# RioWong/PointCloudProcess

Hardware: AMD Instinct MI355X
Metric: Mcorrespondences/s + ICP iter/s, 50M-vs-50M fp32 @ 1/2/4/8 MI355X (higher is better)
Workload: dtype f32

## Files before the change

include/pcp.h:

```cpp
#ifndef PCP_H
#define PCP_H

#include <stddef.h>
#include <stdint.h>

#ifdef __cplusplus
extern "C" {
#endif

#define PCP_ABI_VERSION 1

enum pcp_status {
    PCP_OK = 0,
    PCP_ERR_ARG = -1,
    PCP_ERR_HIP = -2,
    PCP_ERR_NOMEM = -3,
    PCP_ERR_EMPTY = -4,
    PCP_ERR_UNSUPPORTED = -5,
    PCP_ERR_ICP = -6,
    PCP_ERR_CAPACITY = -7
};

#define PCP_AOS48_STRIDE 48

// ... 121 lines not shown
#define PCP_ICP_ABLATE_NO_FALLBACK 8
#define PCP_ICP_ABLATE_NO_VERIFY 64
#define PCP_ICP_OPT_WIDE_CACHE 128
#define PCP_ICP_OPT_GRAPH 256
#define PCP_ICP_OPT_NO_LOOKAHEAD 512
int pcp_icp_set_options(pcp_icp* icp, int oct_lanes_first, int oct_lanes_list, int ring_lanes, int ablate);
int pcp_icp_destroy(pcp_icp* icp);
int pcp_icp_step(pcp_ctx* ctx, pcp_icp* icp, const double T_host[16], float rmax,
                 double* acc_dev, int32_t* corr_idx_dev, float* corr_d2_dev);
int pcp_icp_keys(pcp_ctx* ctx, pcp_icp* icp, const double T_host[16], float rmax,
                 int64_t target_offset, uint64_t* keys_dev);
int pcp_icp_accumulate_keys(pcp_ctx* ctx, pcp_icp* icp, const double T_host[16],
                            const uint64_t* keys_dev, int64_t lo, int64_t hi,
                            const float* shard_xyz_dev, size_t shard_stride_bytes,
                            double* acc_dev);
int pcp_icp_keys_dev(pcp_ctx* ctx, pcp_icp* icp, const double* T_dev, float rmax,
                     int64_t target_offset, uint64_t* keys_dev);
int pcp_keys_owner(pcp_ctx* ctx, const uint64_t* keys_dev, int64_t n, const int64_t* bounds_dev, int nshards,
                   uint8_t* owner_dev);
int pcp_icp_accumulate_owned(pcp_ctx* ctx, const double* T_dev, const float* q_dev, size_t q_stride_bytes,
                             int64_t nq, const uint64_t* keys_dev, const uint8_t* owner_dev, int rank,
                             int64_t lo, int64_t hi, const float* shard_xyz_dev, size_t shard_stride_bytes,
                             double* acc_dev);
int pcp_slab_guard(pcp_ctx* ctx, const double* T_dev, const double box_host[6], double lo,
                   double hi, int* flag_dev);
int pcp_icp_solve(const double acc_host[24], int do_scale, double dT_host[16]);
int pcp_icp_run(pcp_ctx* ctx, pcp_icp* icp, double T_inout[16], float rmax, int iters,
                int do_scale, double eps, float* err);
int pcp_icp_last_kernel_ms(const pcp_icp* icp, double* ms, int* launches);
int pcp_icp_step_dev(pcp_ctx* ctx, pcp_icp* icp, const double* T_dev, float rmax, double* acc_dev);
int pcp_icp_solve_dev(pcp_ctx* ctx, const double* acc_dev, int do_scale, double* T_dev, double* stats_dev);
int pcp_icp_run_dev(pcp_ctx* ctx, pcp_icp* icp, double* T_dev, float rmax, int iters, int do_scale,
                    double* stats_dev);
int pcp_icp_kernel_ms(pcp_ctx* ctx, pcp_icp* icp, double* ms, int* launches);
int pcp_icp_last_fallback(const pcp_icp* icp, int64_t* n);
int pcp_icp_last_searched(const pcp_icp* icp, int64_t* n);
int pcp_icp_last_lookahead(const pcp_icp* icp, double* beta, double* max_offset_m);

int pcp_get_rot_icp(pcp_ctx* ctx, const void* src_aos48_dev, int64_t ns, int src_is_dense,
                    const void* temp_aos48_dev, int64_t nt, int temp_is_dense,
                    double mat_rot_host[16], float rmax, int iters, int do_scale,
                    double cell_size, float* err);

#define PCP_ICP_PLANE_ACC 30
typedef struct pcp_icp_planes pcp_icp_planes;

int pcp_icp_planes_create(pcp_ctx* ctx, const float* target_xyz_dev, size_t t_stride_bytes,
                          const float* normals_dev, size_t n_stride_bytes, int64_t n,
                          pcp_icp_planes** out);
int pcp_icp_planes_destroy(pcp_icp_planes* planes);
int64_t pcp_icp_planes_size(const pcp_icp_planes* planes);
int64_t pcp_icp_planes_valid(const pcp_icp_planes* planes);

int pcp_icp_accumulate_plane(pcp_ctx* ctx, const double* T_dev, const float* q_dev, size_t q_stride_bytes,
                             int64_t nq, const uint64_t* keys_dev, const pcp_icp_planes* planes,
                             double* acc_dev );
int pcp_icp_solve_plane(const double acc_host[30], double dT_host[16]);
int pcp_icp_solve_plane_dev(pcp_ctx* ctx, const double* acc_dev, double* T_dev, double* stats_dev );
int pcp_icp_run_plane_dev(pcp_ctx* ctx, pcp_icp* icp, const pcp_icp_planes* planes, const float* q_dev,
                          size_t q_stride_bytes, int64_t nq, double* T_dev, float rmax, int iters,
                          double* stats_dev);
int pcp_get_rot_icp_plane(pcp_ctx* ctx, const void* src_aos48_dev, int64_t ns, int src_is_dense,
                          const void* temp_aos48_dev, int64_t nt, int temp_is_dense,
                          double mat_rot_host[16], float rmax, int iters, int normals_k,
                          double cell_size, float* err);

// ... 75 lines not shown
```

pointcloudprocess_amd/_lib.py:

```python
import ctypes as C
import os

HERE = os.path.dirname(os.path.abspath(__file__))
_AB = os.environ.get("PCP_AB") == "1" and bool(os.environ.get("PCP_LIB"))
LIB_PATH = os.environ["PCP_LIB"] if _AB else os.path.join(HERE, "libpcp.so")

PCP_OK = 0
_STATUS = {
    -1: "PCP_ERR_ARG", -2: "PCP_ERR_HIP", -3: "PCP_ERR_NOMEM", -4: "PCP_ERR_EMPTY",
    -5: "PCP_ERR_UNSUPPORTED", -6: "PCP_ERR_ICP", -7: "PCP_ERR_CAPACITY",
}

_vp, _i32, _i64, _sz, _f32, _f64, _u32 = (C.c_void_p, C.c_int, C.c_int64, C.c_size_t,
                                          C.c_float, C.c_double, C.c_uint32)
_P = C.POINTER
SIGNATURES = [
    ("pcp_abi_version", _i32, []),
    ("pcp_ctx_create", _i32, [_i32, _vp, _P(_vp)]),
    ("pcp_ctx_destroy", _i32, [_vp]),
    ("pcp_ctx_set_stream", _i32, [_vp, _vp]),
    ("pcp_ctx_stream", _vp, [_vp]),
    ("pcp_last_error", C.c_char_p, [_vp]),
    ("pcp_sync", _i32, [_vp]),
    ("pcp_ctx_alloc_stats", _i32, [_vp, _vp]),
# ... 38 lines not shown
    ("pcp_grid_create", _i32, [_vp, _P(_vp)]),
    ("pcp_grid_destroy", _i32, [_vp]),
    ("pcp_grid_clear", _i32, [_vp, _vp]),
    ("pcp_grid_add_cloud", _i32, [_vp, _vp, _vp, _i64]),
    ("pcp_grid_size", _i64, [_vp]),
    ("pcp_grid_cells", _i64, [_vp]),
    ("pcp_grid_last_dedupe", _i32, [_vp, _P(_i64)]),
    ("pcp_grid_points", _i32, [_vp, _vp, _vp, _i64, _P(_i64)]),
    ("pcp_grid_box", _i32, [_vp, _vp, _i32, _i32, _i32, _i32, _vp, _i64, _P(_i64)]),
    ("pcp_grid_match", _i32, [_vp, _vp, _vp, _i64, _f32, _vp, _P(_i64), _vp, _i64, _P(_i64)]),
    ("pcp_pose_lum_elch", _i32, [_vp, _i64, _i64, _i64, _vp]),
    ("pcp_pose_loop_closure", _i32, [_vp, _vp, _i64, _vp, _vp, _i64, _i64]),
    ("pcp_remove_duplicate", _i32, [_vp, _vp, _i64, _i32, _f32, _vp, _P(_i64)]),
    ("pcp_normals_knn", _i32, [_vp, _vp, _i32, _vp, _i64]),
    ("pcp_normals_knn_last_deferred", _i32, [_vp, _P(_i64), _P(_i64)]),
    ("pcp_icp_create", _i32, [_vp, _vp, _vp, _sz, _i64, _P(_vp)]),
    ("pcp_icp_check_sizes", _i32, [_i64, _i64]),
    ("pcp_icp_destroy", _i32, [_vp]),
    ("pcp_icp_create_with_target", _i32, [_vp, _vp, _sz, _i64, _f64, _vp, _sz, _i64, _P(_vp), _P(_vp)]),
    ("pcp_icp_set_options", _i32, [_vp, _i32, _i32, _i32, _i32]),
    ("pcp_icp_step", _i32, [_vp, _vp, _P(_f64), _f32, _vp, _vp, _vp]),
    ("pcp_icp_keys", _i32, [_vp, _vp, _P(_f64), _f32, _i64, _vp]),
    ("pcp_icp_accumulate_keys", _i32, [_vp, _vp, _P(_f64), _vp, _i64, _i64, _vp, _sz, _vp]),
    ("pcp_icp_keys_dev", _i32, [_vp, _vp, _vp, _f32, _i64, _vp]),
    ("pcp_keys_owner", _i32, [_vp, _vp, _i64, _vp, _i32, _vp]),
    ("pcp_icp_accumulate_owned", _i32, [_vp, _vp, _vp, _sz, _i64, _vp, _vp, _i32, _i64, _i64, _vp, _sz, _vp]),
    ("pcp_slab_guard", _i32, [_vp, _vp, _P(_f64), _f64, _f64, _vp]),
    ("pcp_icp_solve", _i32, [_P(_f64), _i32, _P(_f64)]),
    ("pcp_icp_run", _i32, [_vp, _vp, _P(_f64), _f32, _i32, _i32, _f64, _P(_f32)]),
    ("pcp_icp_last_kernel_ms", _i32, [_vp, _P(_f64), _P(_i32)]),
    ("pcp_icp_step_dev", _i32, [_vp, _vp, _vp, _f32, _vp]),
    ("pcp_icp_solve_dev", _i32, [_vp, _vp, _i32, _vp, _vp]),
    ("pcp_icp_run_dev", _i32, [_vp, _vp, _vp, _f32, _i32, _i32, _vp]),
    ("pcp_icp_kernel_ms", _i32, [_vp, _vp, _P(_f64), _P(_i32)]),
    ("pcp_icp_last_fallback", _i32, [_vp, _P(_i64)]),
    ("pcp_icp_last_searched", _i32, [_vp, _P(_i64)]),
    ("pcp_icp_last_lookahead", _i32, [_vp, _P(_f64), _P(_f64)]),
    ("pcp_fault_report_install", _i32, []),
    ("pcp_build_id", C.c_char_p, []),
    ("pcp_get_rot_icp", _i32, [_vp, _vp, _i64, _i32, _vp, _i64, _i32, _P(_f64), _f32, _i32, _i32,
                               _f64, _P(_f32)]),
    ("pcp_icp_planes_create", _i32, [_vp, _vp, _sz, _vp, _sz, _i64, _P(_vp)]),
    ("pcp_icp_planes_destroy", _i32, [_vp]),
    ("pcp_icp_planes_size", _i64, [_vp]),
    ("pcp_icp_planes_valid", _i64, [_vp]),
    ("pcp_icp_accumulate_plane", _i32, [_vp, _vp, _vp, _sz, _i64, _vp, _vp, _vp]),
    ("pcp_icp_solve_plane", _i32, [_P(_f64), _P(_f64)]),
    ("pcp_icp_solve_plane_dev", _i32, [_vp, _vp, _vp, _vp]),
    ("pcp_icp_run_plane_dev", _i32, [_vp, _vp, _vp, _vp, _sz, _i64, _vp, _f32, _i32, _vp]),
    ("pcp_get_rot_icp_plane", _i32, [_vp, _vp, _i64, _i32, _vp, _i64, _i32, _P(_f64), _f32, _i32, _i32,
                                     _f64, _P(_f32)]),
    ("pcp_icp_trim_keys", _i32, [_vp, _vp, _i64, _f32, _f32, _f32, _vp, _vp]),
    ("pcp_icp_run_plane_trimmed_dev", _i32, [_vp, _vp, _vp, _vp, _sz, _i64, _vp, _f32, _f32, _f32, _f32, _i32,
                                             _vp, _vp]),
    ("pcp_get_rot_icp_plane_trimmed", _i32, [_vp, _vp, _i64, _i32, _vp, _i64, _i32, _P(_f64), _f32, _f32, _f32,
                                             _f32, _i32, _i32, _f64, _P(_f32), _P(_i64)]),
    ("pcp_icp_trim_keys_plane", _i32, [_vp, _vp, _vp, _sz, _i64, _vp, _vp, _f32, _f32, _f32, _vp, _vp]),
    ("pcp_icp_run_plane_rtrimmed_dev", _i32, [_vp, _vp, _vp, _vp, _sz, _i64, _vp, _f32, _f32, _f32, _f32, _i32,
                                              _vp, _vp]),
    ("pcp_get_rot_icp_plane_rtrimmed", _i32, [_vp, _vp, _i64, _i32, _vp, _i64, _i32, _P(_f64), _f32, _f32, _f32,
                                              _f32, _i32, _i32, _f64, _P(_f32), _P(_i64)]),
    ("pcp_icp_batch_create", _i32, [_vp, _vp, _vp, _sz, _i64, _P(_i64), _i32, _P(_vp)]),
    ("pcp_icp_batch_destroy", _i32, [_vp]),
    ("pcp_icp_batch_queries", _i64, [_vp]),
    ("pcp_icp_batch_segments", _i32, [_vp]),
    ("pcp_icp_batch_keys_dev", _i32, [_vp, _vp, _vp, _f32, _vp]),
# ... 54 lines not shown
```

pointcloudprocess_amd/csrc/icp.hip:

```cpp
#include <cmath>
#include <cstdlib>
#include <cstring>
#include <vector>

#include <rocprim/device/device_select.hpp>
#include <rocprim/iterator/counting_iterator.hpp>
#include "sortcfg.hpp"

#include "icp_pair.hpp"
#include "wave_acc.hpp"

namespace pcp {
struct QXyz {
    float x, y, z;
};
}

struct pcp_icp {
    pcp_ctx* ctx = nullptr;
    pcp_ctx* owner = nullptr;
    const pcp_index* target = nullptr;
    int64_t nq = 0;
    int64_t nq_in = 0;
    pcp::QXyz* q = nullptr;
// ... 1037 lines not shown
        ring_run<2>(a, s_acc, list, list_n);
    else if (G == 4)
        ring_run<4>(a, s_acc, list, list_n);
    else
        ring_run<8>(a, s_acc, list, list_n);
    write_wave_partials(s_acc, partials + (int64_t)blockIdx.x * kAcc);
}

__global__ void __launch_bounds__(256) k_list_compact(const int32_t* __restrict__ seg, const uint32_t* __restrict__ cnt,
                                                      int64_t nseg, int64_t seg_cap, int32_t* __restrict__ out,
                                                      uint32_t* __restrict__ total) {
    __shared__ uint32_t s_part[4];
    const int lane = threadIdx.x & 63, w = threadIdx.x >> 6;
    const int64_t s0 = (int64_t)blockIdx.x * 4;
    uint32_t acc = 0;
    for (int64_t i = threadIdx.x; i < s0; i += 256) acc += cnt[i];
    for (int o = 32; o > 0; o >>= 1) acc += (uint32_t)__shfl_xor((int)acc, o, 64);
    if (lane == 0) s_part[w] = acc;
    __syncthreads();
    const uint32_t base = s_part[0] + s_part[1] + s_part[2] + s_part[3];
    uint32_t c[4];
#pragma unroll
    for (int k = 0; k < 4; k++) c[k] = s0 + k < nseg ? cnt[s0 + k] : 0u;
    uint32_t off = base;
#pragma unroll
    for (int k = 0; k < 3; k++) off += k < w ? c[k] : 0u;
    const int64_t sg = s0 + w;
    if (sg < nseg)
        for (uint32_t k = (uint32_t)lane; k < c[w]; k += 64) out[off + k] = seg[sg * seg_cap + k];
    if (s0 + 4 >= nseg && threadIdx.x == 0) *total = base + c[0] + c[1] + c[2] + c[3];
}

constexpr int kRedGroups = 32;
__global__ void __launch_bounds__(kAcc * kRedGroups) k_reduce_partials(const double* __restrict__ part, int nb,
                                                                       double* out, const uint32_t* fb_total) {
    __shared__ double s[kRedGroups][kAcc];
    const int k = threadIdx.x % kAcc, grp = threadIdx.x / kAcc;
    double v = 0.0;
    int b = grp;
    for (; b + 7 * kRedGroups < nb; b += 8 * kRedGroups) {
        double x[8];
#pragma unroll
        for (int u = 0; u < 8; u++) x[u] = part[(int64_t)(b + u * kRedGroups) * kAcc + k];
#pragma unroll
        for (int u = 0; u < 8; u++) v += x[u];
    }
    for (; b < nb; b += kRedGroups) v += part[(int64_t)b * kAcc + k];
    s[grp][k] = v;
    __syncthreads();
    if (threadIdx.x < kAcc) {
        double t = 0.0;
        for (int j = 0; j < kRedGroups; j++) t += s[j][threadIdx.x];
        out[threadIdx.x] = threadIdx.x == kAcc - 1 ? (fb_total ? (double)*fb_total : 0.0) : t;
    }
}

__global__ void k_scatter_corr(IcpArgs a, int32_t* idx, float* d2) {
    load_pose(a);
    for (int64_t i = blockIdx.x * (int64_t)blockDim.x + threadIdx.x; i < a.nq;
         i += (int64_t)gridDim.x * blockDim.x) {
        const float4 qq = ldq(a, i);
        const int oq = a.qidx[i];
        float x, y, z;
        xform(a, qq, x, y, z);
        const CacheBest w = cache_best(a.tp, cache_load(a, i), x, y, z);
        const bool ok = w.bd <= a.r2;
        idx[oq] = ok ? w.bj : -1;
        d2[oq] = ok ? w.bd : INFINITY;
    }
}

__global__ void k_fill_corr(int32_t* idx, float* d2, int64_t n) {
    for (int64_t i = blockIdx.x * (int64_t)blockDim.x + threadIdx.x; i < n;
         i += (int64_t)gridDim.x * blockDim.x) {
        idx[i] = -1;
        d2[i] = INFINITY;
    }
}

__global__ void k_fill_keys(uint64_t* keys, int64_t n) {
    for (int64_t i = blockIdx.x * (int64_t)blockDim.x + threadIdx.x; i < n; i += (int64_t)gridDim.x * blockDim.x)
        keys[i] = kNoKey;
}

__global__ void k_make_keys(IcpArgs a, uint32_t offset, uint64_t* keys) {
    load_pose(a);
    for (int64_t i = blockIdx.x * (int64_t)blockDim.x + threadIdx.x; i < a.nq; i += (int64_t)gridDim.x * blockDim.x) {
// ... 42 lines not shown
            while (hi - lo > 1) {
                const int mid = (lo + hi) >> 1;
                if (bounds[mid] <= g) lo = mid;
                else hi = mid;
            }
            o = (uint8_t)lo;
        }
        owner[i] = o;
    }
}

__global__ void __launch_bounds__(kPairBlock) k_acc_owned(const double* T, const float* q, size_t qs, int64_t n,
                                                          const uint64_t* keys, const uint8_t* owner, int rank,
                                                          int64_t lo, int64_t hi, const float* shard, size_t ss,
                                                          double* partials) {
    const Pose32 P = pose32(T);
    double acc[kAcc - 1];
#pragma unroll
    for (int k = 0; k < kAcc - 1; k++) acc[k] = 0.0;
    for (int64_t i = blockIdx.x * (int64_t)blockDim.x + threadIdx.x; i < n; i += (int64_t)gridDim.x * blockDim.x) {
        if (owner[i] != (uint8_t)rank) continue;
        const uint64_t key = keys[i];
        const int64_t g = (int64_t)key_index(key);
        if (key == kNoKey || g < lo || g >= hi) continue;
        const float* p = shard + (size_t)(g - lo) * ss;
        float x, y, z;
        xform(P, q + (size_t)i * qs, x, y, z);
        const double qv[3] = {x, y, z}, pv[3] = {p[0], p[1], p[2]};
        kabsch_terms(qv, pv, key, acc);
    }
    block_partials<kAcc - 1, kAcc>(acc, partials + (int64_t)blockIdx.x * kAcc);
}

__global__ void k_slab_guard(const double* T, double b0, double b1, double b2, double b3, double b4, double b5,
                             double lo, double hi, int* flag) {
    const double bx[2] = {b0, b1}, by[2] = {b2, b3}, bz[2] = {b4, b5};
    double mn = INFINITY, mx = -INFINITY;
    for (int c = 0; c < 8; c++) {
        const double x = T[0] * bx[c & 1] + T[1] * by[(c >> 1) & 1] + T[2] * bz[c >> 2] + T[3];
        mn = fmin(mn, x);
        mx = fmax(mx, x);
    }
    if (!(mn >= lo && mx <= hi)) *flag = 1;
}

__global__ void k_query_keys(GridDesc g, const float* q, size_t stride_f, int64_t n, uint32_t* key, float4* rec) {
    for (int64_t i = blockIdx.x * (int64_t)blockDim.x + threadIdx.x; i < n; i += (int64_t)gridDim.x * blockDim.x) {
        const float* p = q + (size_t)i * stride_f;
        const float x = p[0], y = p[1], z = p[2];
        const bool fin = isfinite(x) && isfinite(y) && isfinite(z);
        uint32_t k = query_key_end(g);
        if (fin) k = query_cell_key(g, x, y, z);
        key[i] = k;
        rec[i] = make_float4(x, y, z, __int_as_float((int)i));
    }
}

__global__ void k_split_queries(const float4* qs, int64_t n, QXyz* q, int32_t* qi) {
    for (int64_t i = blockIdx.x * (int64_t)blockDim.x + threadIdx.x; i < n; i += (int64_t)gridDim.x * blockDim.x) {
        const float4 v = qs[i];
        q[i] = QXyz{v.x, v.y, v.z};
        qi[i] = __float_as_int(v.w);
    }
}

__global__ void k_first_at_least(const uint32_t* sorted, int64_t n, uint32_t key, unsigned long long* out) {
    int64_t lo = 0, hi = n;
    while (lo < hi) {
        const int64_t mid = (lo + hi) >> 1;
        if (sorted[mid] < key) lo = mid + 1;
        else hi = mid;
    }
    *out = (unsigned long long)lo;
}

__host__ __device__ void svd3(const double Ain[9], double U[9], double s[3], double V[9]) {
    double A[9];
// ... 46 lines not shown
    const double tiny = 1e-14 * (s[0] > 0 ? s[0] : 1.0);
    for (int c = 0; c < 3; c++)
        for (int r = 0; r < 3; r++) U[3 * r + c] = s[c] > tiny ? A2[3 * r + c] / s[c] : 0.0;
    if (!(s[2] > tiny)) {
        double u0[3] = {U[0], U[3], U[6]}, u1[3] = {U[1], U[4], U[7]};
        if (!(s[1] > tiny)) {
            double a[3] = {fabs(u0[0]) < 0.9 ? 1.0 : 0.0, fabs(u0[0]) < 0.9 ? 0.0 : 1.0, 0.0};
            double d = a[0] * u0[0] + a[1] * u0[1] + a[2] * u0[2];
            for (int r = 0; r < 3; r++) u1[r] = a[r] - d * u0[r];
            double nn = sqrt(u1[0] * u1[0] + u1[1] * u1[1] + u1[2] * u1[2]);
            for (int r = 0; r < 3; r++) { u1[r] /= nn; U[3 * r + 1] = u1[r]; }
        }
        double u2[3] = {u0[1] * u1[2] - u0[2] * u1[1], u0[2] * u1[0] - u0[0] * u1[2], u0[0] * u1[1] - u0[1] * u1[0]};
        for (int r = 0; r < 3; r++) U[3 * r + 2] = u2[r];
    }
}

__host__ __device__ double det3(const double M[9]) {
    return M[0] * (M[4] * M[8] - M[5] * M[7]) - M[1] * (M[3] * M[8] - M[5] * M[6]) +
           M[2] * (M[3] * M[7] - M[4] * M[6]);
}

}

struct LookAhead {
    float lo[3], hi[3];
    float alpha, cap;
    int off;
};
#ifndef PCP_LOOK_ALPHA
#define PCP_LOOK_ALPHA 0.5f
#endif
constexpr float kLookAlpha = PCP_LOOK_ALPHA, kLookCap = 0.02f, kLookRmax = 0.9f;
__global__ void k_pose_set(const double* T, Pose32 hp, LookAhead la, float* pose, float* hist, uint32_t launch) {
    *(uint32_t*)(pose + 24) = launch;
    for (int k = 0; k < 12; k++) pose[12 + k] = pose[k];
    for (int r = 0; r < 3; r++) {
        for (int c = 0; c < 3; c++) pose[3 * r + c] = T ? (float)T[4 * r + c] : hp.R[3 * r + c];
        pose[9 + r] = T ? (float)T[4 * r + 3] : hp.t[r];
    }
    double A[9], B[9], ta[3], tb[3], Ai[9], BA[9], v[3];
    for (int k = 0; k < 9; k++) { A[k] = pose[k]; B[k] = pose[12 + k]; }
    for (int k = 0; k < 3; k++) { ta[k] = pose[9 + k]; tb[k] = pose[21 + k]; }
    const double det = det3(A);
    Ai[0] = A[4] * A[8] - A[5] * A[7]; Ai[1] = A[2] * A[7] - A[1] * A[8]; Ai[2] = A[1] * A[5] - A[2] * A[4];
    Ai[3] = A[5] * A[6] - A[3] * A[8]; Ai[4] = A[0] * A[8] - A[2] * A[6]; Ai[5] = A[2] * A[3] - A[0] * A[5];
    Ai[6] = A[3] * A[7] - A[4] * A[6]; Ai[7] = A[1] * A[6] - A[0] * A[7]; Ai[8] = A[0] * A[4] - A[1] * A[3];
    for (int r = 0; r < 3; r++)
        for (int c = 0; c < 3; c++)
            BA[3 * r + c] = (B[3 * r] * Ai[c] + B[3 * r + 1] * Ai[3 + c] + B[3 * r + 2] * Ai[6 + c]) / det;
    for (int r = 0; r < 3; r++) v[r] = BA[3 * r] * ta[0] + BA[3 * r + 1] * ta[1] + BA[3 * r + 2] * ta[2] - tb[r];
    double s2 = 0.0;
    for (int c = 0; c < 8; c++) {
        const double y[3] = {c & 1 ? la.hi[0] : la.lo[0], c & 2 ? la.hi[1] : la.lo[1], c & 4 ? la.hi[2] : la.lo[2]};
        double d2 = 0.0;
        for (int r = 0; r < 3; r++) {
            const double d = y[r] - (BA[3 * r] * y[0] + BA[3 * r + 1] * y[1] + BA[3 * r + 2] * y[2]) + v[r];
            d2 += d * d;
        }
        s2 = fmax(s2, d2);
    }
    const float step = launch > 0 ? (float)sqrt(s2) : 0.f, prev = pose[kPoseStep];
    float beta = 0.f;
    const float ratio = launch == 1 ? 0.f : (prev > 0.f ? step / prev : 0.f);
    if (!la.off && launch > 0 && step > 0.f && ratio > 0.f && ratio < 1.f) {
        const float r = fminf(ratio, kLookRmax);
        beta = la.alpha * r / (1.f - r);
        if (beta * step > la.cap) beta = la.cap / step;
    }
    pose[kPoseStep] = step;
    pose[kPoseBeta] = beta;
    pose[kPoseOff] = beta * step;
    for (int k = 0; k < 12; k++) pose[kPoseC + k] = __fmaf_rn(beta, pose[k] - pose[12 + k], pose[k]);
    for (int k = 0; k < 12; k++) hist[k] = pose[kPoseC + k];
}

__host__ __device__ int icp_solve(const double acc[24], int do_scale, double dT[16]);

__global__ void k_icp_solve_dev(const double* acc, int do_scale, double* T, double* stats) {
    if (stats[0] < 0) return;
    double a[24], dT[16], Tn[16];
    for (int k = 0; k < 24; k++) a[k] = acc[k];
    stats[2] += a[23];
    if (icp_solve(a, do_scale, dT) != PCP_OK) {
        stats[0] = -1.0;
        return;
    }
    stats[1] = sqrt(a[22] / a[0]);
    stats[3] += 1.0;
    for (int i = 0; i < 4; i++)
        for (int j = 0; j < 4; j++) {
            double v = 0;
            for (int k = 0; k < 4; k++) v += dT[4 * i + k] * T[4 * k + j];
            Tn[4 * i + j] = v;
        }
    for (int k = 0; k < 16; k++) T[k] = Tn[k];
}

using OctKernel = void (*)(IcpArgs, const int32_t*, const uint32_t*);
int icp_chain(pcp_icp* icp, hipStream_t st, IcpArgs& a, OctKernel oct) {
    pcp_ctx* ctx = icp->ctx;
    uint32_t* const svc_n = icp->sv_off + a.nseg_v;
    uint32_t* const fbc_n = icp->fb_off + a.nseg;
    a.partials = icp->partials;
    hipLaunchKernelGGL(k_icp_verify, dim3(icp->nb_ver), dim3(kIcpBlock), 0, st, a);
    hipLaunchKernelGGL(k_list_compact, dim3((unsigned)((a.nseg_v + 3) / 4)), dim3(256), 0, st,
                       (const int32_t*)icp->sv, (const uint32_t*)icp->sv_count, a.nseg_v, a.sv_seg, icp->svc, svc_n);
    if (icp->dbg) PCP_HIP(ctx, hipEventRecord(icp->ev_ver, st));
    a.partials += (int64_t)icp->nb_ver * kAcc;
    hipLaunchKernelGGL(oct, dim3(icp->nb_fast_l), dim3(kIcpBlock), 0, st, a, (const int32_t*)icp->svc,
                       (const uint32_t*)svc_n);
    if (icp->dbg) PCP_HIP(ctx, hipEventRecord(icp->ev_mid, st));
    hipLaunchKernelGGL(k_list_compact, dim3((unsigned)((a.nseg + 3) / 4)), dim3(256), 0, st,
                       (const int32_t*)icp->fb, (const uint32_t*)icp->fb_count, a.nseg, a.fb_seg, icp->fbc, fbc_n);
    a.partials += (int64_t)icp->nb_fast * kAcc;
    hipLaunchKernelGGL(k_icp_ring, dim3(icp->nb_ring), dim3(kIcpBlock), 0, st, a, a.partials,
                       (const int32_t*)icp->fbc, (const uint32_t*)fbc_n);
    return PCP_OK;
}

int icp_launch(pcp_icp* icp, const double T[16], float rmax, double* acc_dev, int32_t* corr_idx,
               float* corr_d2, const double* T_dev = nullptr, IcpArgs* args_out = nullptr) {
    pcp_ctx* ctx = icp->ctx;
    const pcp_index* tg = icp->target;
    IcpArgs a{};
    a.g = tg->g;
    a.tp = (const float4*)tg->pts;
    a.q = icp->q;
    a.qidx = icp->qidx;
    a.nq = icp->nq;
    a.nchunks = (icp->nq + kIcpBlock - 1) / kIcpBlock;
    const Pose32 hp = T_dev ? Pose32{} : pose32(T);
    LookAhead la{};
    for (int k = 0; k < 3; k++) {
        la.lo[k] = (float)(a.g.o[k] - rmax);
        la.hi[k] = (float)(a.g.o[k] + a.g.n[k] * a.g.h + rmax);
    }
    la.alpha = kLookAlpha;
    la.cap = kLookCap;
    la.off = icp->no_look ? 1 : 0;
    hipLaunchKernelGGL(k_pose_set, dim3(1), dim3(1), 0, ctx->stream, T_dev, hp, la, icp->pose_dev,
                       icp->pose_hist + (icp->launches & (icp->narrow ? 63 : kHist - 1)) * 12,
                       (uint32_t)icp->launches);
    a.pose = icp->pose_dev;
    a.launch_dev = (const uint32_t*)(icp->pose_dev + 24);
    for (int k = 0; k < 9; k++) a.R[k] = hp.R[k];
    for (int k = 0; k < 3; k++) a.t[k] = hp.t[k];
    a.r2 = rmax * rmax;
    a.mc = search_margin(a.g);
    a.rho = 0.5f;
    const double rr = (0.5 - (double)a.mc) * a.g.h;
    a.cert2 = (float)(rr * rr * (1.0 - 1e-5));
    a.cand = icp->cand;
    a.narrow = icp->narrow ? 1 : 0;
    a.hist_mask = icp->narrow ? 63u : (uint32_t)(kHist - 1);
    a.max_age = icp->narrow ? 32u : 128u;
    a.dunit = (float)(a.g.h / 1024.0);
    a.inv_dunit = (float)(1024.0 / a.g.h);
    a.pose_hist = icp->pose_hist;
    a.launch = (uint32_t)icp->launches;
    a.ntp = (uint32_t)tg->n;
    a.sv = icp->sv;
    a.sv_count = icp->sv_count;
    a.sv_off = icp->sv_off;
    a.sv_seg = icp->sv_seg;
    a.nseg_v = icp->nseg_v;
    a.fb = icp->fb;
    a.fb_count = icp->fb_count;
    a.fb_off = icp->fb_off;
    a.fb_seg = icp->fb_seg;
    a.nb_fast = icp->nb_fast;
    a.nseg = (int64_t)icp->nb_fast * (kIcpBlock / 64);
    a.ring_all = a.g.dense ? 0 : 1;
    a.dbg = icp->dbg;
    double* part_v = icp->partials;
    double* part_o = part_v + (int64_t)icp->nb_ver * kAcc;
// ... 41 lines not shown
            if (e == hipSuccess) e = hipGraphInstantiate(&icp->gexec, gr, nullptr, nullptr, 0);
            if (gr) (void)hipGraphDestroy(gr);
            if (e != hipSuccess) {
                icp->gexec = nullptr;
                icp->graph_off = true;
                (void)hipGetLastError();
            }
            icp->graph_r2 = a.r2;
        }
        if (graph && icp->gexec) PCP_HIP(ctx, hipGraphLaunch(icp->gexec, ctx->stream));
        else PCP_TRY(icp_chain(icp, ctx->stream, a, oct_list));
    } else {
        const int nb_idle = a.g.dense ? icp->nb_ver : icp->nb_ver + icp->nb_fast;
        PCP_HIP(ctx, hipMemsetAsync(part_v, 0, (size_t)nb_idle * kAcc * sizeof(double), ctx->stream));
        if (a.g.dense) {
            if (icp->dbg) PCP_HIP(ctx, hipEventRecord(icp->ev_ver, ctx->stream));
            a.partials = part_o;
            a.oct_g = icp->oct_g_first;
            hipLaunchKernelGGL((k_icp_octant<PCP_OCT_WAVES, false>), dim3(icp->nb_fast), dim3(kIcpBlock), 0,
                               ctx->stream, a, (const int32_t*)nullptr, (const uint32_t*)nullptr);
        }
        if (icp->dbg) PCP_HIP(ctx, hipEventRecord(icp->ev_mid, ctx->stream));
        if (a.g.dense) {
            hipLaunchKernelGGL(k_list_compact, dim3((unsigned)((a.nseg + 3) / 4)), dim3(256), 0, ctx->stream,
                               (const int32_t*)icp->fb, (const uint32_t*)icp->fb_count, a.nseg, a.fb_seg, icp->fbc,
                               icp->fb_off + a.nseg);
        }
        a.partials = part_r;
        a.ring_g = icp->ring_g;
        hipLaunchKernelGGL(k_icp_ring, dim3(icp->nb_ring), dim3(kIcpBlock), 0, ctx->stream, a, part_r,
                           (const int32_t*)icp->fbc, (const uint32_t*)(icp->fb_off + a.nseg));
    }
    PCP_HIP(ctx, hipEventRecord(e1, ctx->stream));
    hipLaunchKernelGGL(k_reduce_partials, dim3(1), dim3(kAcc * kRedGroups), 0, ctx->stream, icp->partials,
                       icp->nb_ver + icp->nb_fast + icp->nb_ring, acc_dev,
                       a.g.dense ? (const uint32_t*)(icp->fb_off + a.nseg) : nullptr);
    if (corr_idx) {
        if (icp->nq_in > icp->nq)
            hipLaunchKernelGGL(k_fill_corr, dim3(grid_for(icp->nq_in, 256)), dim3(256), 0, ctx->stream, corr_idx,
                               corr_d2, icp->nq_in);
        if (icp->nq > 0)
            hipLaunchKernelGGL(k_scatter_corr, dim3(grid_for(icp->nq, 256)), dim3(256), 0, ctx->stream, a,
                               corr_idx, corr_d2);
    }
    if (args_out) *args_out = a;
    icp->launches++;
    PCP_LAUNCH_CHECK(ctx);
    return PCP_OK;
}

__host__ __device__ int icp_solve(const double acc[24], int do_scale, double dT[16]) {
    const double n = acc[0];
    if (!(n >= 3.0)) return PCP_ERR_ICP;
    double qm[3], pm[3], S[9];
    for (int k = 0; k < 3; k++) { qm[k] = acc[1 + k] / n; pm[k] = acc[4 + k] / n; }
    for (int a = 0; a < 3; a++)
        for (int b = 0; b < 3; b++) S[3 * a + b] = acc[7 + 3 * a + b] - n * qm[a] * pm[b];
    double U[9], s[3], V[9];
    svd3(S, U, s, V);
    double R[9];
    for (int a = 0; a < 3; a++)
        for (int b = 0; b < 3; b++) {
            double v = 0;
            for (int k = 0; k < 3; k++) v += V[3 * a + k] * U[3 * b + k];
            R[3 * a + b] = v;
        }
    double d = det3(R) < 0 ? -1.0 : 1.0;
    if (d < 0) {
        for (int a = 0; a < 3; a++)
// ... 382 lines not shown
    if (n == 0) return PCP_OK;
    hipLaunchKernelGGL(pcp::k_keys_owner, dim3(pcp::grid_for(n, 256, 8192)), dim3(256), 0, ctx->stream, keys_dev, n,
                       bounds_dev, nshards, owner_dev);
    PCP_LAUNCH_CHECK(ctx);
    return PCP_OK;
}

int pcp_icp_accumulate_owned(pcp_ctx* ctx, const double* T_dev, const float* q_dev, size_t q_stride, int64_t nq,
                             const uint64_t* keys_dev, const uint8_t* owner_dev, int rank, int64_t lo, int64_t hi,
                             const float* shard_xyz_dev, size_t shard_stride, double* acc_dev) {
    if (!ctx || !T_dev || nq < 0 || (nq > 0 && (!q_dev || !keys_dev || !owner_dev)) || !acc_dev || rank < 0 ||
        rank > 254 || lo < 0 || hi < lo || (hi > lo && !shard_xyz_dev))
        return PCP_ERR_ARG;
    if (q_stride == 0) q_stride = 3 * sizeof(float);
    if (shard_stride == 0) shard_stride = 3 * sizeof(float);
    if (q_stride % sizeof(float) || shard_stride % sizeof(float))
        return pcp::set_error(ctx, PCP_ERR_ARG, "strides must be whole floats");
    PCP_HIP(ctx, hipSetDevice(ctx->device));
    const int nb = (int)std::min<int64_t>(std::max<int64_t>(1, (nq + 255) / 256), 2048);
    pcp::Tmp tmp(ctx);
    double* part = nullptr;
    PCP_TRY(tmp.get(&part, (size_t)nb * pcp::kAcc));
    const dim3 block(pcp::kPairBlock);
    hipLaunchKernelGGL(pcp::k_acc_owned, dim3(nb), block, 0, ctx->stream, T_dev, q_dev, q_stride / sizeof(float), nq,
                       keys_dev, owner_dev, rank, lo, hi, shard_xyz_dev, shard_stride / sizeof(float), part);
    hipLaunchKernelGGL(pcp::k_sum_partials, dim3(1), block, 0, ctx->stream, (const double*)part, nb, acc_dev);
    PCP_LAUNCH_CHECK(ctx);
    return PCP_OK;
}

int pcp_slab_guard(pcp_ctx* ctx, const double* T_dev, const double box[6], double lo, double hi, int* flag_dev) {
    if (!ctx || !T_dev || !box || !flag_dev) return PCP_ERR_ARG;
    PCP_HIP(ctx, hipSetDevice(ctx->device));
    hipLaunchKernelGGL(pcp::k_slab_guard, dim3(1), dim3(1), 0, ctx->stream, T_dev, box[0], box[1], box[2], box[3],
                       box[4], box[5], lo, hi, flag_dev);
    PCP_LAUNCH_CHECK(ctx);
    return PCP_OK;
}

int pcp_icp_accumulate_keys(pcp_ctx* ctx, pcp_icp* icp, const double T[16], const uint64_t* keys_dev,
                            int64_t lo, int64_t hi, const float* shard_xyz_dev, size_t shard_stride_bytes,
                            double* acc_dev) {
    if (!ctx || !icp || !T || !keys_dev || !acc_dev || lo < 0 || hi < lo || (hi > lo && !shard_xyz_dev))
        return PCP_ERR_ARG;
    if (shard_stride_bytes == 0) shard_stride_bytes = 3 * sizeof(float);
    if (shard_stride_bytes % sizeof(float)) return pcp::set_error(ctx, PCP_ERR_ARG, "shard stride must be whole floats");
    PCP_HIP(ctx, hipSetDevice(ctx->device));
    const int nb = (int)std::min<int64_t>(std::max<int64_t>(1, (icp->nq + 255) / 256), icp->nb_fast + icp->nb_ring);
    const dim3 block(pcp::kPairBlock);
    hipLaunchKernelGGL(pcp::k_acc_keys, dim3(nb), block, 0, ctx->stream, icp->q, icp->qidx, icp->nq, keys_dev,
                       (uint64_t)lo, (uint64_t)hi, shard_xyz_dev, shard_stride_bytes / sizeof(float), pcp::pose32(T),
                       icp->partials);
    hipLaunchKernelGGL(pcp::k_sum_partials, dim3(1), block, 0, ctx->stream, (const double*)icp->partials, nb, acc_dev);
    PCP_LAUNCH_CHECK(ctx);
    return PCP_OK;
}

int pcp_icp_solve(const double acc[24], int do_scale, double dT[16]) {
    if (!acc || !dT) return PCP_ERR_ARG;
    return pcp::icp_solve(acc, do_scale, dT);
}

int pcp_icp_run(pcp_ctx* ctx, pcp_icp* icp, double T[16], float rmax, int iters, int do_scale, double eps,
                float* err) {
    if (!ctx || !icp || !T || iters < 0) return PCP_ERR_ARG;
    PCP_HIP(ctx, hipSetDevice(ctx->device));
    icp->ctx = ctx;
    double e = -1.0, ms_total = 0.0;
// ... 115 lines not shown
```

pointcloudprocess_amd/distributed.py:

```python
import math

import numpy as np
import torch
import torch.distributed as dist

from . import ops


def _world():
    return dist.get_world_size() if (dist.is_available() and dist.is_initialized()) else 1


def _allreduce(t, op):
    if _world() > 1:
        if t.is_cuda and dist.get_backend() == "gloo":
            h = t.cpu()
            dist.all_reduce(h, op=op)
            t.copy_(h)
        else:
            dist.all_reduce(t, op=op)
    return t


def _finish(acc_t, T, do_scale):
# ... 89 lines not shown
            ev = (torch.cuda.Event(enable_timing=True), torch.cuda.Event(enable_timing=True))
            ev[0].record()
        _reduce_scatter_min(mine, keys.clone() if keys.device.type == "cpu" else keys)
        engine.key_owner(mine, bnd, own_mine)
        _all_gather_bytes(owner, own_mine)
        if ev is not None:
            ev[1].record()
            exchange.append(ev)
        acc = engine.accumulate_owned(T_dev, keys, owner, rank, lo, hi)
        _allreduce(acc, dist.ReduceOp.SUM)
        engine.solve_dev(acc, T_dev, stats, do_scale)
    st = stats.cpu().numpy()
    T = T_dev.cpu().numpy().reshape(4, 4)
    return (float(st[1]) if st[0] == 0 and st[3] == iters else -1.0), T


def slab_bounds(x, world):
    xs = np.sort(np.asarray(x, dtype=np.float64))
    b = [-np.inf]
    for r in range(1, world):
        b.append(float(xs[(len(xs) * r) // world]) if len(xs) else 0.0)
    b.append(np.inf)
    return b


def slab_select(q_x, t_x, bounds, rank, halo):
    lo, hi = bounds[rank], bounds[rank + 1]
    return (q_x >= lo) & (q_x < hi), (t_x >= lo - halo) & (t_x < hi + halo)


def run_slab_dev(engine, T0, rmax, iters, guard=None, do_scale=False, exchange=None, out_stats=None):
    T_dev, stats = engine.new_pose(T0)
    flag = torch.zeros(1, dtype=torch.int32, device=T_dev.device)
    for _ in range(iters):
        if guard is not None:
            engine.slab_guard(T_dev, guard[0], guard[1], guard[2], flag)
        acc = engine.step_dev(T_dev, rmax)
        ev = None
        if exchange is not None and T_dev.is_cuda:
            ev = (torch.cuda.Event(enable_timing=True), torch.cuda.Event(enable_timing=True))
            ev[0].record()
        _allreduce(acc, dist.ReduceOp.SUM)
        if ev is not None:
            ev[1].record()
            exchange.append(ev)
        engine.solve_dev(acc, T_dev, stats, do_scale)
    ns = stats.numel()
    host = torch.cat([stats.reshape(-1).double(), T_dev.reshape(-1).double(), flag.double()]).cpu().numpy()
    st, T, ok = host[:ns], host[ns:ns + 16].reshape(4, 4).copy(), bool(host[ns + 16] == 0)
    if out_stats is not None:
        out_stats["fallback"] = float(st[2])
    return (float(st[1]) if st[0] == 0 and st[3] == iters else -1.0), T, ok


def shard_range(n, world, rank):
    lo = (n * rank) // world
    return lo, (n * (rank + 1)) // world


class GpuEngine:

    lane_options = None
    graph = False

    def __init__(self, ctx, target_xyz, query_xyz, cell_size=0.0):
        self.target = target_xyz.contiguous()
        if hasattr(ctx.lib, "pcp_icp_create_with_target"):
            self.icp = ops.ICP.with_target(ctx, self.target, query_xyz.contiguous(), cell_size)
            self.index = self.icp.index
        else:
            self.index = ops.GridIndex(ctx, self.target, cell_size=cell_size)
            self.icp = ops.ICP(self.index, query_xyz.contiguous())
        if GpuEngine.lane_options is not None or GpuEngine.graph:
            self.icp.set_options(*(GpuEngine.lane_options or (1, 0, 0)), graph=GpuEngine.graph)
        self.device = ctx.device
        self.nq = query_xyz.shape[0]

    def step(self, T, rmax):
        return self.icp.step(T, rmax)

    def keys(self, T, rmax, offset):
        return self.icp.keys(T, rmax, offset)

    def new_pose(self, T0):
        return self.icp.new_pose(T0)

    def step_dev(self, T_dev, rmax):
        return self.icp.step_dev(T_dev, rmax)

    def solve_dev(self, acc, T_dev, stats, do_scale=False):
        self.icp.solve_dev(acc, T_dev, stats, do_scale)

    def accumulate_keys(self, T, keys, lo, hi):
        return self.icp.accumulate_keys(T, keys, lo, hi, self.target)

    def keys_dev(self, T_dev, rmax, offset, out=None):
        return self.icp.keys_dev(T_dev, rmax, offset, out)

    def key_owner(self, keys, bounds, out):
        return ops.keys_owner(self.index.ctx, keys, bounds, out)

    def accumulate_owned(self, T_dev, keys, owner, rank, lo, hi):
        return ops.accumulate_owned(self.index.ctx, T_dev, self.icp.q, keys, owner, rank, lo, hi, self.target,
                                    self.icp.acc)

    def slab_guard(self, T_dev, box, lo, hi, flag):
        ops.slab_guard(self.index.ctx, T_dev, box, lo, hi, flag)

    def close(self):
        self.icp.close()
        self.index.close()


def radius_slab_split(x, world, rank, r):
    b = slab_bounds(x, world)
    lo, hi = b[rank], b[rank + 1]
    x = np.asarray(x)
    own = np.nonzero((x >= lo) & (x < hi))[0]
    halo = np.nonzero(((x >= lo - r) & (x < lo)) | ((x >= hi) & (x < hi + r)))[0]
    return own, halo


def radius_slab_split_dev(x, world, rank, r):
    n = x.numel()
    xs = torch.sort(x.double()).values
    b = [-math.inf] + [float(xs[(n * k) // world]) if n else 0.0 for k in range(1, world)] + [math.inf]
    del xs
    lo, hi = b[rank], b[rank + 1]
    xd = x.double()
    own = torch.nonzero((xd >= lo) & (xd < hi)).flatten()
    halo = torch.nonzero(((xd >= lo - r) & (xd < lo)) | ((xd >= hi) & (xd < hi + r))).flatten()
    return own, halo


def radius_rows_slab(engine, xyz, r, world=None, rank=None):
    world = _world() if world is None else world
    rank = (dist.get_rank() if world > 1 else 0) if rank is None else rank
    own, halo = radius_slab_split(np.asarray(xyz)[:, 0], world, rank, r)
    gid = np.concatenate([own, halo]).astype(np.int32)
    offs, idx = engine.radius_rows(np.asarray(xyz)[gid], len(own), gid, r)
# ... 2 lines not shown
```

pointcloudprocess_amd/ops.py:

```python
import ctypes as C

import numpy as np
import torch

from . import _lib
from ._lib import check

POINT48 = np.dtype(
    [("x", "<f8"), ("y", "<f8"), ("z", "<f8"), ("w", "<f8"), ("rgba", "<u4"),
     ("stamp_id", "<u4"), ("pad", "<u4", (2,))])
PLANE = np.dtype([("normal_x", "<f4"), ("normal_y", "<f4"), ("normal_z", "<f4"),
                  ("min_value", "<f4"), ("curvature", "<f4"), ("distance", "<f4")])


def _ptr(t):
    return C.c_void_p(t.data_ptr()) if t is not None else None


class Context:

    def __init__(self, device=0):
        self.lib = _lib.load()
        self.device = torch.device("cuda", device) if isinstance(device, int) else torch.device(device)
        idx = self.device.index or 0
# ... 320 lines not shown
            cd = torch.empty(self.q.shape[0], dtype=torch.float32, device=ctx.device)
        ctx.check(ctx.lib.pcp_icp_step(ctx.h, self.h, Tm, float(rmax), _ptr(self.acc), _ptr(ci), _ptr(cd)))
        return (self.acc, ci, cd) if corr else self.acc

    def run(self, T0, rmax, iters, do_scale=False, eps=0.0):
        ctx = self.ctx
        T = _lib.f64arr(np.asarray(T0, dtype=np.float64).reshape(16))
        err = C.c_float()
        rc = ctx.lib.pcp_icp_run(ctx.h, self.h, T, float(rmax), int(iters), int(do_scale), float(eps),
                                 C.byref(err))
        if rc not in (0, -6):
            ctx.check(rc)
        return float(err.value), np.array(T[:]).reshape(4, 4)

    def new_pose(self, T0=None):
        T = torch.as_tensor(np.eye(4) if T0 is None else np.asarray(T0, dtype=np.float64), dtype=torch.float64)
        return T.reshape(16).to(self.ctx.device).contiguous(), torch.zeros(4, dtype=torch.float64,
                                                                        device=self.ctx.device)

    def step_dev(self, T_dev, rmax):
        ctx = self.ctx
        ctx.check(ctx.lib.pcp_icp_step_dev(ctx.h, self.h, _ptr(T_dev), float(rmax), _ptr(self.acc)))
        return self.acc

    def solve_dev(self, acc, T_dev, stats, do_scale=False):
        ctx = self.ctx
        ctx.check(ctx.lib.pcp_icp_solve_dev(ctx.h, _ptr(acc), int(do_scale), _ptr(T_dev), _ptr(stats)))

    def run_dev(self, T_dev, stats, rmax, iters, do_scale=False):
        ctx = self.ctx
        ctx.check(ctx.lib.pcp_icp_run_dev(ctx.h, self.h, _ptr(T_dev), float(rmax), int(iters), int(do_scale),
                                          _ptr(stats)))

    def solve_plane_dev(self, acc, T_dev, stats):
        ctx = self.ctx
        assert acc.dtype == torch.float64 and acc.numel() >= 30
        ctx.check(ctx.lib.pcp_icp_solve_plane_dev(ctx.h, _ptr(acc), _ptr(T_dev), _ptr(stats)))

    def run_plane_dev(self, planes, q, T_dev, stats, rmax, iters):
        ctx = self.ctx
        n = q.shape[0]
        ctx.check(ctx.lib.pcp_icp_run_plane_dev(ctx.h, self.h, planes.h, _ptr(q) if n else None,
                                                q.stride(0) * q.element_size(), n, _ptr(T_dev), float(rmax),
                                                int(iters), _ptr(stats)))

    def run_plane_trimmed_dev(self, planes, q, T_dev, stats, rmax, frac, mult=1.0, d_floor=0.0, iters=4, trim=None):
        ctx = self.ctx
        n = q.shape[0]
        trim = torch.zeros(4, dtype=torch.int64, device=ctx.device) if trim is None else trim
        assert trim.dtype == torch.int64 and trim.numel() >= 4
        ctx.check(ctx.lib.pcp_icp_run_plane_trimmed_dev(ctx.h, self.h, planes.h, _ptr(q) if n else None,
                                                        q.stride(0) * q.element_size(), n, _ptr(T_dev), float(rmax),
                                                        float(frac), float(mult), float(d_floor), int(iters),
                                                        _ptr(stats), _ptr(trim)))
        return trim

    def run_plane_rtrimmed_dev(self, planes, q, T_dev, stats, rmax, frac, mult=1.0, d_floor=0.0, iters=4, trim=None):
        ctx = self.ctx
        n = q.shape[0]
        trim = torch.zeros(4, dtype=torch.int64, device=ctx.device) if trim is None else trim
        assert trim.dtype == torch.int64 and trim.numel() >= 4
        ctx.check(ctx.lib.pcp_icp_run_plane_rtrimmed_dev(ctx.h, self.h, planes.h, _ptr(q) if n else None,
                                                         q.stride(0) * q.element_size(), n, _ptr(T_dev), float(rmax),
                                                         float(frac), float(mult), float(d_floor), int(iters),
                                                         _ptr(stats), _ptr(trim)))
        return trim
# ... 267 lines not shown
```

Before: 29270.

## Fuse ICP reduce, solve, slab guard and pose update into one tail kernel

Adds a device-side slab ICP loop whose per-iteration tail is one kernel. It reduces the partials, solves the pose update, applies the slab guard and precomputes the next pose with look-ahead, replacing several single-thread launches and the Python per-iteration step/solve calls. The Python slab runner uses this path when world size is 1. The cost targeted is kernel launch and host round-trip overhead per ICP iteration. The reduction unroll also goes from 8 to 16, and the serial single-thread tail now sits on the critical path of one bigger block.

```diff
diff --git a/include/pcp.h b/include/pcp.h
--- a/include/pcp.h
+++ b/include/pcp.h
@@ -177,6 +177,9 @@
 int pcp_icp_solve_dev(pcp_ctx* ctx, const double* acc_dev, int do_scale, double* T_dev, double* stats_dev);
 int pcp_icp_run_dev(pcp_ctx* ctx, pcp_icp* icp, double* T_dev, float rmax, int iters, int do_scale,
                     double* stats_dev);
+int pcp_icp_run_slab_dev(pcp_ctx* ctx, pcp_icp* icp, double* T_dev, float rmax, int iters, int do_scale,
+                         const double box_host[6], double lo, double hi, int* flag_dev, double* acc_dev,
+                         double* stats_dev);
 int pcp_icp_kernel_ms(pcp_ctx* ctx, pcp_icp* icp, double* ms, int* launches);
 int pcp_icp_last_fallback(const pcp_icp* icp, int64_t* n);
 int pcp_icp_last_searched(const pcp_icp* icp, int64_t* n);
diff --git a/pointcloudprocess_amd/_lib.py b/pointcloudprocess_amd/_lib.py
--- a/pointcloudprocess_amd/_lib.py
+++ b/pointcloudprocess_amd/_lib.py
@@ -94,6 +94,7 @@
     ("pcp_icp_step_dev", _i32, [_vp, _vp, _vp, _f32, _vp]),
     ("pcp_icp_solve_dev", _i32, [_vp, _vp, _i32, _vp, _vp]),
     ("pcp_icp_run_dev", _i32, [_vp, _vp, _vp, _f32, _i32, _i32, _vp]),
+    ("pcp_icp_run_slab_dev", _i32, [_vp, _vp, _vp, _f32, _i32, _i32, _P(_f64), _f64, _f64, _vp, _vp, _vp]),
     ("pcp_icp_kernel_ms", _i32, [_vp, _vp, _P(_f64), _P(_i32)]),
     ("pcp_icp_last_fallback", _i32, [_vp, _P(_i64)]),
     ("pcp_icp_last_searched", _i32, [_vp, _P(_i64)]),
diff --git a/pointcloudprocess_amd/csrc/icp.hip b/pointcloudprocess_amd/csrc/icp.hip
--- a/pointcloudprocess_amd/csrc/icp.hip
+++ b/pointcloudprocess_amd/csrc/icp.hip
@@ -1093,18 +1093,18 @@
 }
 
 constexpr int kRedGroups = 32;
-__global__ void __launch_bounds__(kAcc * kRedGroups) k_reduce_partials(const double* __restrict__ part, int nb,
-                                                                       double* out, const uint32_t* fb_total) {
-    __shared__ double s[kRedGroups][kAcc];
+template <int U>
+__device__ __forceinline__ void reduce_partials(const double* __restrict__ part, int nb, double* out,
+                                                const uint32_t* fb_total, double (*s)[kAcc], double* tot) {
     const int k = threadIdx.x % kAcc, grp = threadIdx.x / kAcc;
     double v = 0.0;
     int b = grp;
-    for (; b + 7 * kRedGroups < nb; b += 8 * kRedGroups) {
-        double x[8];
-#pragma unroll
-        for (int u = 0; u < 8; u++) x[u] = part[(int64_t)(b + u * kRedGroups) * kAcc + k];
-#pragma unroll
-        for (int u = 0; u < 8; u++) v += x[u];
+    for (; b + (U - 1) * kRedGroups < nb; b += U * kRedGroups) {
+        double x[U];
+#pragma unroll
+        for (int u = 0; u < U; u++) x[u] = part[(int64_t)(b + u * kRedGroups) * kAcc + k];
+#pragma unroll
+        for (int u = 0; u < U; u++) v += x[u];
     }
     for (; b < nb; b += kRedGroups) v += part[(int64_t)b * kAcc + k];
     s[grp][k] = v;
@@ -1112,8 +1112,16 @@
     if (threadIdx.x < kAcc) {
         double t = 0.0;
         for (int j = 0; j < kRedGroups; j++) t += s[j][threadIdx.x];
-        out[threadIdx.x] = threadIdx.x == kAcc - 1 ? (fb_total ? (double)*fb_total : 0.0) : t;
-    }
+        if (threadIdx.x == kAcc - 1) t = fb_total ? (double)*fb_total : 0.0;
+        out[threadIdx.x] = t;
+        if (tot) tot[threadIdx.x] = t;
+    }
+}
+
+__global__ void __launch_bounds__(kAcc * kRedGroups) k_reduce_partials(const double* __restrict__ part, int nb,
+                                                                       double* out, const uint32_t* fb_total) {
+    __shared__ double s[kRedGroups][kAcc];
+    reduce_partials<8>(part, nb, out, fb_total, s, nullptr);
 }
 
 __global__ void k_scatter_corr(IcpArgs a, int32_t* idx, float* d2) {
@@ -1222,9 +1230,14 @@
     block_partials<kAcc - 1, kAcc>(acc, partials + (int64_t)blockIdx.x * kAcc);
 }
 
-__global__ void k_slab_guard(const double* T, double b0, double b1, double b2, double b3, double b4, double b5,
-                             double lo, double hi, int* flag) {
-    const double bx[2] = {b0, b1}, by[2] = {b2, b3}, bz[2] = {b4, b5};
+struct SlabGuard {
+    double b[6], lo, hi;
+    int* flag;
+};
+__device__ __forceinline__ void slab_guard(const double* T, const SlabGuard& g) {
+    const double bx[2] = {g.b[0], g.b[1]}, by[2] = {g.b[2], g.b[3]}, bz[2] = {g.b[4], g.b[5]};
+    const double lo = g.lo, hi = g.hi;
+    int* const flag = g.flag;
     double mn = INFINITY, mx = -INFINITY;
     for (int c = 0; c < 8; c++) {
         const double x = T[0] * bx[c & 1] + T[1] * by[(c >> 1) & 1] + T[2] * bz[c >> 2] + T[3];
@@ -1233,6 +1246,7 @@
     }
     if (!(mn >= lo && mx <= hi)) *flag = 1;
 }
+__global__ void k_slab_guard(const double* T, SlabGuard g) { slab_guard(T, g); }
 
 __global__ void k_query_keys(GridDesc g, const float* q, size_t stride_f, int64_t n, uint32_t* key, float4* rec) {
     for (int64_t i = blockIdx.x * (int64_t)blockDim.x + threadIdx.x; i < n; i += (int64_t)gridDim.x * blockDim.x) {
@@ -1345,7 +1359,8 @@
 #define PCP_LOOK_ALPHA 0.5f
 #endif
 constexpr float kLookAlpha = PCP_LOOK_ALPHA, kLookCap = 0.02f, kLookRmax = 0.9f;
-__global__ void k_pose_set(const double* T, Pose32 hp, LookAhead la, float* pose, float* hist, uint32_t launch) {
+__device__ __forceinline__ void pose_set(const double* T, const Pose32& hp, const LookAhead& la, float* pose,
+                                         float* hist, uint32_t launch) {
     *(uint32_t*)(pose + 24) = launch;
     for (int k = 0; k < 12; k++) pose[12 + k] = pose[k];
     for (int r = 0; r < 3; r++) {
@@ -1387,10 +1402,13 @@
     for (int k = 0; k < 12; k++) pose[kPoseC + k] = __fmaf_rn(beta, pose[k] - pose[12 + k], pose[k]);
     for (int k = 0; k < 12; k++) hist[k] = pose[kPoseC + k];
 }
+__global__ void k_pose_set(const double* T, Pose32 hp, LookAhead la, float* pose, float* hist, uint32_t launch) {
+    pose_set(T, hp, la, pose, hist, launch);
+}
 
 __host__ __device__ int icp_solve(const double acc[24], int do_scale, double dT[16]);
 
-__global__ void k_icp_solve_dev(const double* acc, int do_scale, double* T, double* stats) {
+__device__ __forceinline__ void solve_dev(const double* acc, int do_scale, double* T, double* stats) {
     if (stats[0] < 0) return;
     double a[24], dT[16], Tn[16];
     for (int k = 0; k < 24; k++) a[k] = acc[k];
@@ -1408,6 +1426,30 @@
             Tn[4 * i + j] = v;
         }
     for (int k = 0; k < 16; k++) T[k] = Tn[k];
+}
+__global__ void k_icp_solve_dev(const double* acc, int do_scale, double* T, double* stats) {
+    solve_dev(acc, do_scale, T, stats);
+}
+
+struct IcpTail {
+    int do_scale, next;
+    double *T, *stats;
+    SlabGuard guard;
+    LookAhead la;
+    float *pose, *hist;
+    uint32_t launch;
+};
+__global__ void __launch_bounds__(kAcc * kRedGroups) k_icp_tail(const double* __restrict__ part, int nb, double* out,
+                                                                const uint32_t* fb_total, IcpTail t) {
+    __shared__ double s[kRedGroups][kAcc];
+    __shared__ double tot[kAcc];
+    reduce_partials<16>(part, nb, out, fb_total, s, tot);
+    __syncthreads();
+    if (threadIdx.x != 0) return;
+    solve_dev(tot, t.do_scale, t.T, t.stats);
+    if (!t.next) return;
+    if (t.guard.flag) slab_guard(t.T, t.guard);
+    pose_set(t.T, Pose32{}, t.la, t.pose, t.hist, t.launch);
 }
 
 using OctKernel = void (*)(IcpArgs, const int32_t*, const uint32_t*);
@@ -1432,8 +1474,14 @@
     return PCP_OK;
 }
 
+struct SlabLoop {
+    IcpTail tail;
+    bool pose_preset;
+};
+
 int icp_launch(pcp_icp* icp, const double T[16], float rmax, double* acc_dev, int32_t* corr_idx,
-               float* corr_d2, const double* T_dev = nullptr, IcpArgs* args_out = nullptr) {
+               float* corr_d2, const double* T_dev = nullptr, IcpArgs* args_out = nullptr,
+               SlabLoop* loop = nullptr) {
     pcp_ctx* ctx = icp->ctx;
     const pcp_index* tg = icp->target;
     IcpArgs a{};
@@ -1452,9 +1500,10 @@
     la.alpha = kLookAlpha;
     la.cap = kLookCap;
     la.off = icp->no_look ? 1 : 0;
-    hipLaunchKernelGGL(k_pose_set, dim3(1), dim3(1), 0, ctx->stream, T_dev, hp, la, icp->pose_dev,
-                       icp->pose_hist + (icp->launches & (icp->narrow ? 63 : kHist - 1)) * 12,
-                       (uint32_t)icp->launches);
+    const int64_t hmask = icp->narrow ? 63 : kHist - 1;
+    if (!(loop && loop->pose_preset))
+        hipLaunchKernelGGL(k_pose_set, dim3(1), dim3(1), 0, ctx->stream, T_dev, hp, la, icp->pose_dev,
+                           icp->pose_hist + (icp->launches & hmask) * 12, (uint32_t)icp->launches);
     a.pose = icp->pose_dev;
     a.launch_dev = (const uint32_t*)(icp->pose_dev + 24);
     for (int k = 0; k < 9; k++) a.R[k] = hp.R[k];
@@ -1562,9 +1611,20 @@
                            (const int32_t*)icp->fbc, (const uint32_t*)(icp->fb_off + a.nseg));
     }
     PCP_HIP(ctx, hipEventRecord(e1, ctx->stream));
-    hipLaunchKernelGGL(k_reduce_partials, dim3(1), dim3(kAcc * kRedGroups), 0, ctx->stream, icp->partials,
-                       icp->nb_ver + icp->nb_fast + icp->nb_ring, acc_dev,
-                       a.g.dense ? (const uint32_t*)(icp->fb_off + a.nseg) : nullptr);
+    const uint32_t* const fb_total = a.g.dense ? (const uint32_t*)(icp->fb_off + a.nseg) : nullptr;
+    const int nb_rows = icp->nb_ver + icp->nb_fast + icp->nb_ring;
+    if (loop) {
+        IcpTail& t = loop->tail;
+        t.la = la;
+        t.pose = icp->pose_dev;
+        t.hist = icp->pose_hist + ((icp->launches + 1) & hmask) * 12;
+        t.launch = (uint32_t)(icp->launches + 1);
+        hipLaunchKernelGGL(k_icp_tail, dim3(1), dim3(kAcc * kRedGroups), 0, ctx->stream,
+                           (const double*)icp->partials, nb_rows, acc_dev, fb_total, t);
+    } else {
+        hipLaunchKernelGGL(k_reduce_partials, dim3(1), dim3(kAcc * kRedGroups), 0, ctx->stream, icp->partials,
+                           nb_rows, acc_dev, fb_total);
+    }
     if (corr_idx) {
         if (icp->nq_in > icp->nq)
             hipLaunchKernelGGL(k_fill_corr, dim3(grid_for(icp->nq_in, 256)), dim3(256), 0, ctx->stream, corr_idx,
@@ -2013,8 +2073,33 @@
 int pcp_slab_guard(pcp_ctx* ctx, const double* T_dev, const double box[6], double lo, double hi, int* flag_dev) {
     if (!ctx || !T_dev || !box || !flag_dev) return PCP_ERR_ARG;
     PCP_HIP(ctx, hipSetDevice(ctx->device));
-    hipLaunchKernelGGL(pcp::k_slab_guard, dim3(1), dim3(1), 0, ctx->stream, T_dev, box[0], box[1], box[2], box[3],
-                       box[4], box[5], lo, hi, flag_dev);
+    hipLaunchKernelGGL(pcp::k_slab_guard, dim3(1), dim3(1), 0, ctx->stream, T_dev,
+                       pcp::SlabGuard{{box[0], box[1], box[2], box[3], box[4], box[5]}, lo, hi, flag_dev});
+    PCP_LAUNCH_CHECK(ctx);
+    return PCP_OK;
+}
+
+int pcp_icp_run_slab_dev(pcp_ctx* ctx, pcp_icp* icp, double* T_dev, float rmax, int iters, int do_scale,
+                         const double box[6], double lo, double hi, int* flag_dev, double* acc_dev,
+                         double* stats_dev) {
+    if (!ctx || !icp || !T_dev || !stats_dev || iters < 0 || !(rmax >= 0.f) || (box && !flag_dev))
+        return PCP_ERR_ARG;
+    PCP_HIP(ctx, hipSetDevice(ctx->device));
+    icp->ctx = ctx;
+    pcp::SlabLoop loop{};
+    pcp::IcpTail& t = loop.tail;
+    t.do_scale = do_scale;
+    t.T = T_dev;
+    t.stats = stats_dev;
+    if (box) t.guard = pcp::SlabGuard{{box[0], box[1], box[2], box[3], box[4], box[5]}, lo, hi, flag_dev};
+    for (int it = 0; it < iters; it++) {
+        if (it == 0 && box)
+            hipLaunchKernelGGL(pcp::k_slab_guard, dim3(1), dim3(1), 0, ctx->stream, (const double*)T_dev, t.guard);
+        loop.pose_preset = it > 0;
+        t.next = it + 1 < iters;
+        PCP_TRY(pcp::icp_launch(icp, nullptr, rmax, acc_dev ? acc_dev : icp->acc, nullptr, nullptr, T_dev, nullptr,
+                                &loop));
+    }
     PCP_LAUNCH_CHECK(ctx);
     return PCP_OK;
 }
diff --git a/pointcloudprocess_amd/distributed.py b/pointcloudprocess_amd/distributed.py
--- a/pointcloudprocess_amd/distributed.py
+++ b/pointcloudprocess_amd/distributed.py
@@ -145,7 +145,10 @@
 def run_slab_dev(engine, T0, rmax, iters, guard=None, do_scale=False, exchange=None, out_stats=None):
     T_dev, stats = engine.new_pose(T0)
     flag = torch.zeros(1, dtype=torch.int32, device=T_dev.device)
-    for _ in range(iters):
+    fused = _world() == 1 and getattr(engine, "fused_slab", False)
+    if fused:
+        engine.run_slab_dev(T_dev, stats, rmax, iters, guard, flag, do_scale)
+    for _ in range(0 if fused else iters):
         if guard is not None:
             engine.slab_guard(T_dev, guard[0], guard[1], guard[2], flag)
         acc = engine.step_dev(T_dev, rmax)
@@ -188,6 +191,7 @@
             self.icp.set_options(*(GpuEngine.lane_options or (1, 0, 0)), graph=GpuEngine.graph)
         self.device = ctx.device
         self.nq = query_xyz.shape[0]
+        self.fused_slab = hasattr(ctx.lib, "pcp_icp_run_slab_dev")
 
     def step(self, T, rmax):
         return self.icp.step(T, rmax)
@@ -219,6 +223,9 @@
 
     def slab_guard(self, T_dev, box, lo, hi, flag):
         ops.slab_guard(self.index.ctx, T_dev, box, lo, hi, flag)
+
+    def run_slab_dev(self, T_dev, stats, rmax, iters, guard, flag, do_scale=False):
+        self.icp.run_slab_dev(T_dev, stats, rmax, iters, guard, flag, do_scale)
 
     def close(self):
         self.icp.close()
diff --git a/pointcloudprocess_amd/ops.py b/pointcloudprocess_amd/ops.py
--- a/pointcloudprocess_amd/ops.py
+++ b/pointcloudprocess_amd/ops.py
@@ -376,6 +376,16 @@
         ctx.check(ctx.lib.pcp_icp_run_dev(ctx.h, self.h, _ptr(T_dev), float(rmax), int(iters), int(do_scale),
                                           _ptr(stats)))
 
+    def run_slab_dev(self, T_dev, stats, rmax, iters, guard=None, flag=None, do_scale=False):
+        ctx = self.ctx
+        box = None if guard is None else _lib.f64arr(np.asarray(guard[0], dtype=np.float64).reshape(6))
+        lo, hi = (0.0, 0.0) if guard is None else (float(guard[1]), float(guard[2]))
+        assert guard is None or (flag is not None and flag.dtype == torch.int32)
+        ctx.check(ctx.lib.pcp_icp_run_slab_dev(ctx.h, self.h, _ptr(T_dev), float(rmax), int(iters), int(do_scale),
+                                               box, lo, hi, _ptr(flag) if guard is not None else None,
+                                               _ptr(self.acc), _ptr(stats)))
+        return self.acc
+
     def solve_plane_dev(self, acc, T_dev, stats):
         ctx = self.ctx
         assert acc.dtype == torch.float64 and acc.numel() >= 30
```

New measurement: 29600, median of 6. +1.1%, better.
